# Elyptos/VolumetricRaytracer

Hardware: AMD Instinct MI355X
Metric: Mrays/sec at 1080p, 256^3 SDF volume (higher is better)
Workload: dtype f32

## Files before the change

include/vrt.h:

```cpp
#ifndef VRT_H
#define VRT_H

#include <stddef.h>
#include <stdint.h>

#ifdef __cplusplus
extern "C" {
#endif

#define VRT_MAX_VOLUMES      20
#define VRT_MAX_POINT_LIGHTS 5
#define VRT_MAX_SPOT_LIGHTS  5
#define VRT_MAX_INSTANCES    64
#define VRT_MAX_DEVICES      8
#define VRT_MAX_RESOLUTION   9
#define VRT_FRAMES_IN_FLIGHT 3
#define VRT_MAX_TEXTURES     64
#define VRT_FLAG_DIAG_TIMELINE 4
#define VRT_FLAG_OUTPUT_RGBA8 8

#define VRT_FLAG_BLOCK_PER_FRAME 64
#define VRT_FLAG_NO_CULL_RECT 128
#define VRT_FLAG_FULL_ONE_KERNEL 256
#define VRT_FLAG_FULL_THREE_PASS 512
#define VRT_FLAG_OUTPUT_BGRA8 2048
#define VRT_FLAG_NO_HIT_POLISH 1024
#define VRT_FLAG_REFERENCE_VIEW_VECTOR 4096
#define VRT_FLAG_REFERENCE_BOUNDARY_TEXELS 8192
#define VRT_HIT_POLISH_SAMPLES 2
#define VRT_FLAG_NO_TIMING 16

enum vrt_status {
    VRT_OK = 0,
    VRT_ERR_INVALID = -1,
    VRT_ERR_NO_DEVICE = -2,
    VRT_ERR_HIP = -3,
    VRT_ERR_OOM = -4,
    VRT_ERR_SLOT = -5,
    VRT_ERR_NOT_READY = -6,
    VRT_ERR_UNSUPPORTED = -7
};

enum vrt_render_mode {
// ... 244 lines not shown

int vrt_last_timing(vrt_ctx* ctx, vrt_timing* out);
int vrt_timing_history(vrt_ctx* ctx, int n, float* kernel_ms_out);

int vrt_launch_history(vrt_ctx* ctx, int n, float* kernel_ms_out, int* frames_out);

long long vrt_debug_wave_records(vrt_ctx* ctx, int which, uint32_t* out, long long max_words);

#define VRT_FORM_FULL 1
#define VRT_FORM_PASSES 2
#define VRT_FORM_TEXTURED 4
#define VRT_FORM_MAY_BOUNCE 8
#define VRT_FORM_LEAN_REF 16
int vrt_debug_last_kernel_form(vrt_ctx* ctx);

int vrt_debug_gather_ceiling(vrt_ctx* ctx, int format, int coherent_lanes, unsigned n_bricks, float* gsamples_per_s_out);

const char* vrt_strerror(int status);
const char* vrt_version(void);

#ifdef __cplusplus
}
#endif
#endif
```

volumetricraytracer_amd/_abi.py:

```python
from __future__ import annotations

import ctypes as C
import os

VRT_MAX_VOLUMES = 20
VRT_MAX_TEXTURES = 64
VRT_FRAMES_IN_FLIGHT = 3
VRT_MAX_RESOLUTION = 9
VRT_MAX_POINT_LIGHTS = 5
VRT_MAX_SPOT_LIGHTS = 5
VRT_MAX_INSTANCES = 64
VRT_MAX_DEVICES = 8
VRT_COMM_ID_BYTES = 128

VRT_OK = 0
VRT_ERR_INVALID = -1
VRT_ERR_NO_DEVICE = -2
VRT_ERR_HIP = -3
VRT_ERR_OOM = -4
VRT_ERR_SLOT = -5
VRT_ERR_NOT_READY = -6
VRT_ERR_UNSUPPORTED = -7

MODE_INTERP = 0
# ... 4 lines not shown
MODE_CUBE_UNLIT = 5
MODE_CUBE_NOTEX = 6
MODE_CUBE_NOTEX_UNLIT = 7

FORM_FULL, FORM_PASSES, FORM_TEXTURED, FORM_MAY_BOUNCE, FORM_LEAN_REF = 1, 2, 4, 8, 16
FLAG_DIAG_TIMELINE = 4
FLAG_OUTPUT_RGBA8 = 8
FLAG_NO_TIMING = 16
FLAG_BLOCK_PER_FRAME = 64
FLAG_NO_CULL_RECT = 128
FLAG_FULL_ONE_KERNEL = 256
FLAG_FULL_THREE_PASS = 512
FLAG_OUTPUT_BGRA8 = 2048
FLAG_REFERENCE_VIEW_VECTOR = 4096
FLAG_REFERENCE_BOUNDARY_TEXELS = 8192
FLAG_NO_HIT_POLISH = 1024
HIT_POLISH_SAMPLES = 2
MAX_BLOCK_FRAMES = 48
MAX_LAUNCH_FRAMES = 256

VOLUME_BYTES_DENSE, VOLUME_BYTES_MATERIAL, VOLUME_BYTES_BRICKS, VOLUME_BYTES_CELLS = 0, 1, 2, 3
VOLUME_BYTES_SKIP, VOLUME_BYTES_NIB, VOLUME_BYTES_CUBE_SKIP, VOLUME_BYTES_ACTIVE_BOX = 4, 5, 6, 7

FORMAT_F32 = 0
FORMAT_TEXEL16 = 1

PATH_AUTO = 0
PATH_DENSE = 1
PATH_BRICK = 2
PATH_BRICK_LDS = 3
# ... 191 lines not shown
    "vrt_comm_init": (C.c_int, [C.c_void_p, C.c_int, C.c_int, C.c_void_p]),
    "vrt_comm_destroy": (C.c_int, [C.c_void_p]),
    "vrt_comm_expect_sizes": (C.c_int, [C.c_void_p, C.c_size_t, C.c_size_t]),
    "vrt_gather_tiles": (C.c_int, [C.c_void_p, C.c_void_p, C.c_void_p, C.c_size_t, C.c_int, C.c_void_p]),
    "vrt_exchange_tiles": (C.c_int, [C.c_void_p, C.c_void_p, C.c_void_p, C.c_size_t, C.c_void_p]),
    "vrt_render_begin": (C.c_int, [C.c_void_p, C.POINTER(vrt_params), C.c_int]),
    "vrt_render_end": (C.c_int, [C.c_void_p, C.c_int, C.POINTER(C.c_void_p)]),
    "vrt_trace_rays": (C.c_int, [C.c_void_p, C.POINTER(vrt_params), C.c_int, C.c_int, C.c_void_p, C.c_void_p, C.c_void_p]),
    "vrt_trace_rays_host": (C.c_int, [C.c_void_p, C.POINTER(vrt_params), C.c_int, C.c_int, C.c_void_p, C.c_void_p]),
    "vrt_camera_rays": (C.c_int, [C.POINTER(vrt_scene), C.c_int, C.c_int, C.c_int, C.c_void_p, C.c_void_p]),
    "vrt_last_timing": (C.c_int, [C.c_void_p, C.POINTER(vrt_timing)]),
    "vrt_timing_history": (C.c_int, [C.c_void_p, C.c_int, C.POINTER(C.c_float)]),
    "vrt_launch_history": (C.c_int, [C.c_void_p, C.c_int, C.POINTER(C.c_float), C.POINTER(C.c_int)]),
    "vrt_debug_wave_records": (C.c_longlong, [C.c_void_p, C.c_int, C.c_void_p, C.c_longlong]),
    "vrt_debug_last_kernel_form": (C.c_int, [C.c_void_p]),
    "vrt_debug_gather_ceiling": (C.c_int, [C.c_void_p, C.c_int, C.c_int, C.c_uint, C.POINTER(C.c_float)]),
    "vrt_strerror": (C.c_char_p, [C.c_int]),
    "vrt_version": (C.c_char_p, []),
}

LIB_PATH = os.path.join(os.path.dirname(os.path.abspath(__file__)), "lib", "libvrt_hip.so")

_lib = None


def _share_hip_runtime_with_torch() -> None:
    import sys

    if "torch" in sys.modules or os.environ.get("VRT_NO_TORCH_PRELOAD") == "1":
        return
# ... 42 lines not shown
```

volumetricraytracer_amd/csrc/host/HipRenderer.cpp:

```cpp
#include "HipRenderer.h"

#include <algorithm>

#include <cmath>
#include <cstdio>
#include <cstdlib>
#include <cstring>
#include <vector>

#include <zlib.h>

#define V_LOG_ERROR(msg) fprintf(stderr, "[VHipRenderer][error] %s\n", (msg))
#define V_LOG_WARNING(msg) fprintf(stderr, "[VHipRenderer][warning] %s\n", (msg))

namespace VolumeRaytracer {

VObjectPtr<VTexture2D> VTexture2D::LoadPPM(const std::string& path) {
    FILE* f = fopen(path.c_str(), "rb");
    if (!f) return nullptr;
    auto token = [&](char* buf, size_t n) {
        int c = fgetc(f);
        while (c != EOF) {
            if (c == '#') {
                while (c != EOF && c != '\n') c = fgetc(f);
// ... 579 lines not shown
    p.max_steps = MaxSteps << std::max(0, MaxResolution - 8);
    p.shadow = Shadows ? 1 : 0;
    p.mode = (int)RenderMode;
    p.path = DataPath;
    p.max_bounces = MaxBounces;
    p.eps_hit = std::min(0.004f * MinCell, 0.02f);
    p.eps_in = 0.01f;
    p.step_min = std::min(0.004f * MinCell, 0.02f);
    p.k_relax = Relaxation;
    const VObjectPtr<Scene::VCamera> cam = scene.GetActiveCamera();
    p.cone_eps = std::tan((cam ? cam->FOVAngle : 60.f) * (3.14159265358979323846f / 180.0f) * 0.5f) / (float)Height;
    if (FrameFormat != EFrameFormat::Float4) p.flags |= VRT_FLAG_OUTPUT_RGBA8;
    if (FrameFormat == EFrameFormat::BGRA8) p.flags |= VRT_FLAG_OUTPUT_BGRA8;
    if (ReferenceViewVector) p.flags |= VRT_FLAG_REFERENCE_VIEW_VECTOR;
    if (ReferenceBoundaryTexels) p.flags |= VRT_FLAG_REFERENCE_BOUNDARY_TEXELS;
    return p;
}

void VHipRenderer::Render() {
    if (!IsActive()) {
        V_LOG_WARNING("Render() on an inactive renderer");
        return;
    }
    const VObjectPtr<Scene::VScene> scene = SceneRef.lock();
    if (!scene) return;
    if (const VObjectPtr<Scene::VCamera> cam = scene->GetActiveCamera()) cam->AspectRatio = (float)Width / (float)Height;
    if (!SyncWithScene(*scene)) return;
    const vrt_params p = MakeParams(*scene);
    const size_t bytes = (size_t)Width * Height * BytesPerPixel();
    if (FramesInFlight <= 1 || Devices.size() != 1) {
// ... 174 lines not shown
```

volumetricraytracer_amd/csrc/host/HipRenderer.h:

```cpp
#pragma once
#include <functional>
#include <map>
#include <string>
#include <vector>
#include "../../../include/vrt.h"
#include "HostRenderer.h"

namespace VolumeRaytracer {
namespace Renderer {
namespace Hip {

class VHipRenderer : public VRenderer {
public:
    VHipRenderer();
    ~VHipRenderer() override;

    void Render() override;
    bool Start() override;
    void Stop() override;
    bool IsActive() const override { return Ctx != nullptr; }
    void InitializeTexture(VObjectPtr<VTexture> texture) override;
    void UploadToGPU(VObjectPtr<VTexture> texture) override;
    void UploadToGPU(VObjectPtr<VTextureCube> texture);
    void UploadToGPU(VObjectPtr<VTexture2D> texture);
// ... 5 lines not shown
    enum class EFrameFormat { Float4, RGBA8, BGRA8 };
    EFrameFormat FrameFormat = EFrameFormat::BGRA8;
    size_t BytesPerPixel() const { return FrameFormat == EFrameFormat::Float4 ? 16 : 4; }
    const void* GetFrameData() const { return FramePixels; }
    size_t GetFrameByteCount() const { return FrameBytes; }
    const float* GetFramePixels() const { return FrameFormat == EFrameFormat::Float4 ? static_cast<const float*>(FramePixels) : nullptr; }
    unsigned GetWidth() const { return Width; }
    unsigned GetHeight() const { return Height; }
    bool GetLastTiming(vrt_timing& out) const;
    int MaxSteps = 255;
    int VolumeFormat = VRT_FORMAT_TEXEL16;
    bool RegionUploads = true;
    bool ReferenceDefaultTextures = true;
    bool ReferenceViewVector = true;
    bool ReferenceBoundaryTexels = true;
    float Relaxation = 1.7f;
    bool Shadows = true;
    int MaxBounces = 2;
    int DataPath = VRT_PATH_AUTO;
    int FramesInFlight = 3;
    void Flush();
    bool RenderBlock(int n_frames, const std::function<void(int)>& tick);
    const void* GetBlockFrame(int f) const { return (BlockFrames && f >= 0 && f < BlockFrameCount) ? BlockFrames + (size_t)f * BlockFrameBytes : nullptr; }
    bool TraceRays(const std::vector<vrt_ray>& rays, std::vector<vrt_hit>& hits, bool anyHit = false);
    bool Pick(int px, int py, vrt_hit& out);
    const Scene::VVoxelObject* HitObject(const vrt_hit& hit) const {
        return hit.instance >= 0 && (size_t)hit.instance < QueryObjects.size() ? QueryObjects[(size_t)hit.instance] : nullptr;
    }

    bool ApplyBrushes(const Scene::VVoxelObject& object, const std::vector<vrt_brush>& brushes, vrt_brush_result* result = nullptr);
// ... 43 lines not shown
```

volumetricraytracer_amd/csrc/vrt_api.hip:

```cpp
#include <hip/hip_runtime.h>

#include <dlfcn.h>
#include <math.h>
#include <stdio.h>
#include <string.h>

#include <algorithm>
#include <chrono>
#include <limits>
#include <new>
#include <vector>

#include "../../include/vrt.h"
#include "vrt_device.h"
#include "vrt_launch.h"
#include "voxelize_core.h"

using namespace vrt;

namespace {

constexpr int kNcclUint8 = 1;
struct RcclApi {
    typedef struct { char internal[VRT_COMM_ID_BYTES]; } UniqueId;
// ... 148 lines not shown
    unsigned* d_diag = nullptr;
    void* edit_staging = nullptr;
    size_t edit_staging_cap = 0;
    void* edit_scratch = nullptr;
    size_t edit_scratch_cap = 0;
    int* d_box6 = nullptr;
    DBrushSlot* d_brush = nullptr;
    void* fill_scratch = nullptr;
    size_t fill_scratch_cap = 0;
    void* query_buf = nullptr;
    size_t query_cap = 0;
    int last_blocks = 0;
    int last_frames = 1;
    bool last_diag = false;
    int last_form = 0;
    hipEvent_t joined = nullptr;
    hipEvent_t ev0[kRing];
    hipEvent_t ev1[kRing];
    FrameSlot slot[VRT_FRAMES_IN_FLIGHT];
    bool events_ok = false;
    int ring_frames[kRing] = {};
    bool timed[kRing] = {};
};

}

struct vrt_ctx {
    std::vector<DeviceState> dev;
    HostVolume vol[VRT_MAX_VOLUMES];
    HostTexture tex[VRT_MAX_TEXTURES];
// ... 805 lines not shown
    }
    return VRT_OK;
}

int check_params(const vrt_ctx* ctx, const vrt_params* p, bool own_scenes = false) {
    if (!ctx || !p) return VRT_ERR_INVALID;
    if (p->width <= 0 || p->height <= 0 || p->width > 16384 || p->height > 16384) return VRT_ERR_INVALID;
    if (p->max_steps < 0 || p->max_steps > 65535 || p->max_bounces < 0 || p->max_bounces > 2) return VRT_ERR_INVALID;
    if (!(p->eps_hit == p->eps_hit) || !(p->step_min > 0.0f) || !(p->k_relax > 0.0f) || !(p->eps_in >= 0.0f) ||
        !(p->cone_eps >= 0.0f))
        return VRT_ERR_INVALID;
    if (p->mode < VRT_MODE_INTERP || p->mode > VRT_MODE_CUBE_NOTEX_UNLIT) return VRT_ERR_INVALID;
    if (p->path < VRT_PATH_AUTO || p->path > VRT_PATH_CELLS) return VRT_ERR_INVALID;
    if ((p->flags & ~(3 | VRT_FLAG_DIAG_TIMELINE | VRT_FLAG_OUTPUT_RGBA8 | VRT_FLAG_NO_TIMING | 32 | VRT_FLAG_BLOCK_PER_FRAME | VRT_FLAG_NO_CULL_RECT |
                      VRT_FLAG_FULL_ONE_KERNEL | VRT_FLAG_FULL_THREE_PASS | VRT_FLAG_NO_HIT_POLISH | VRT_FLAG_OUTPUT_BGRA8 |
                      VRT_FLAG_REFERENCE_VIEW_VECTOR | VRT_FLAG_REFERENCE_BOUNDARY_TEXELS)) != 0 || (p->flags & 3) == 3 ||
        ((p->flags & VRT_FLAG_OUTPUT_BGRA8) && !(p->flags & VRT_FLAG_OUTPUT_RGBA8)) ||
        ((p->flags & VRT_FLAG_FULL_ONE_KERNEL) && (p->flags & VRT_FLAG_FULL_THREE_PASS)))
        return VRT_ERR_INVALID;
    if (!ctx->have_scene && !own_scenes) return VRT_ERR_NOT_READY;
    return VRT_OK;
}

int resolve_path(const vrt_ctx* ctx, int path, bool single, int mode, const vrt_scene* scenes = nullptr, int n_scenes = 0) {
    int n16 = 0, n32 = 0;
    if (!scenes) {
        scenes = &ctx->scene;
        n_scenes = 1;
    }
    for (int f = 0; f < n_scenes; f++)
        for (int i = 0; i < scenes[f].n_instances; i++)
// ... 151 lines not shown
                  : 0;
    F.back = p->mode >= VRT_MODE_CUBE ? 0.2f : 0.1f;
    F.max_bounces = p->max_bounces;
    F.width = p->width;
    F.height = p->height;
    F.row0 = row0;
    F.rows = rows;
    F.tiles_x = (p->width + 15) / 16;
    F.tiles_y = (rows + 15) / 16;
    F.tile_map = p->flags & 3;
    F.diag = (p->flags & VRT_FLAG_DIAG_TIMELINE) ? 1 : 0;
    F.rgba8 = (p->flags & VRT_FLAG_OUTPUT_RGBA8) ? ((p->flags & VRT_FLAG_OUTPUT_BGRA8) ? 2 : 1) : 0;
    F.polish = (p->flags & VRT_FLAG_NO_HIT_POLISH) ? 0 : VRT_HIT_POLISH_SAMPLES;
    F.view_vec = (p->flags & VRT_FLAG_REFERENCE_VIEW_VECTOR) ? 1 : 0;
    F.zero_outside = (p->flags & VRT_FLAG_REFERENCE_BOUNDARY_TEXELS) ? 1 : 0;
    F.strip_rows = rs.strip_rows;
    F.strip_first = rs.strip_first;
    F.strip_stride = rs.strip_stride;
    const ClosestHitForm form = closest_hit_form(ctx, p, scenes, n_scenes);
    F.textured = form.textured ? 1 : 0;
    F.full = form.full ? 1 : 0;
    F.may_bounce = form.may_bounce ? 1 : 0;
    F.n_inst = ctx->scene.n_instances;
    F.n_nodes = ctx->n_nodes;
    F.n_point = std::min(ctx->scene.n_point_lights, VRT_MAX_POINT_LIGHTS);
    F.n_spot = std::min(ctx->scene.n_spot_lights, VRT_MAX_SPOT_LIGHTS);
    F.vols = snapshot ? snapshot->vols : D.d_vols;
    F.inst = snapshot ? snapshot->inst : D.d_inst;
    F.nodes = snapshot ? snapshot->nodes : D.d_nodes;
    F.point = snapshot ? snapshot->point : D.d_point;
// ... 119 lines not shown
    if (passes) {
        const size_t per_frame = (size_t)D.last_blocks * 256, records = per_frame * (size_t)n_frames;
        if (per_frame > 0xffffffffull) return VRT_ERR_INVALID;
        if (D.pass_cap[slot] < records) {
            void* grown = nullptr;
            HIP_TRY(hipMalloc(&grown, records * (sizeof(HitRecord) + sizeof(unsigned)) + records / 64 * sizeof(unsigned long long)));
            if (D.d_pass[slot]) D.pass_retired.push_back(D.d_pass[slot]);
            D.d_pass[slot] = grown;
            D.pass_cap[slot] = records;
        }
        char* base = static_cast<char*>(D.d_pass[slot]);
        F.hit_rec = reinterpret_cast<HitRecord*>(base);
        F.hit_mask = reinterpret_cast<unsigned long long*>(base + D.pass_cap[slot] * sizeof(HitRecord));
        F.hit_aux = reinterpret_cast<unsigned*>(base + D.pass_cap[slot] * sizeof(HitRecord) + D.pass_cap[slot] / 64 * sizeof(unsigned long long));
        F.rec_stride = (uint32_t)per_frame;
    }
    D.last_diag = F.diag != 0;
    D.last_form = (F.full ? VRT_FORM_FULL : 0) | (passes ? VRT_FORM_PASSES : 0) | (F.textured ? VRT_FORM_TEXTURED : 0) |
                  (F.may_bounce ? VRT_FORM_MAY_BOUNCE : 0) | ((!F.full && (F.textured || F.view_vec || F.zero_outside)) ? VRT_FORM_LEAN_REF : 0);
    if (F.diag) {
        if (stat_blocks > (size_t)kMaxBlocks) return VRT_ERR_INVALID;
        if (!D.d_diag) HIP_TRY(hipMalloc(&D.d_diag, sizeof(unsigned) * kDiagRecord * 4 * (size_t)kMaxBlocks));
        F.diag_buf = D.d_diag;
    }
    hipStreamCaptureStatus cap = hipStreamCaptureStatusNone;
    if (stream != nullptr && hipStreamIsCapturing(stream, &cap) != hipSuccess) cap = hipStreamCaptureStatusNone;
    D.timed[ring] = cap == hipStreamCaptureStatusNone && !(p->flags & VRT_FLAG_NO_TIMING);
    D.ring_frames[ring] = n_frames;
    if (D.timed[ring]) HIP_TRY(hipEventRecord(D.ev0[ring], stream));
    HIP_TRY(launch_march(B, path, single, stream));
// ... 958 lines not shown
    } while (false);
    if (e0) (void)hipEventDestroy(e0);
    if (e1) (void)hipEventDestroy(e1);
    if (pool) (void)hipFree(pool);
    if (out) (void)hipFree(out);
    if (rc != VRT_OK) return rc;
    *gsamples_per_s_out = (float)((double)blocks * 256.0 * iters / ((double)best * 1e6));
    return VRT_OK;
}

int vrt_debug_last_kernel_form(vrt_ctx* ctx) {
    if (!ctx || ctx->dev.empty()) return VRT_ERR_INVALID;
    return ctx->dev[0].last_form;
}

long long vrt_debug_wave_records(vrt_ctx* ctx, int which, uint32_t* out, long long max_words) {
    if (!ctx || max_words < 0 || (max_words > 0 && !out) || which < 0 || which > 3) return VRT_ERR_INVALID;
    if (ctx->launches == 0) return VRT_ERR_NOT_READY;
    DeviceState& D = ctx->dev[0];
    const bool diag = (which & 1) != 0, whole = which >= 2;
    if (diag && (!D.last_diag || !D.d_diag)) return VRT_ERR_NOT_READY;
    const long long frame_words = (long long)D.last_blocks * 4 * (diag ? kDiagRecord : kStatRecord);
    const long long words = whole ? frame_words * D.last_frames : frame_words;
    if (out && max_words > 0) {
        HIP_TRY(hipSetDevice(D.ordinal));
        HIP_TRY(hipDeviceSynchronize());
        const uint32_t* src = (diag ? D.d_diag : D.d_stats[D.last_slot]) + (whole ? 0 : (size_t)(D.last_frames - 1) * (size_t)frame_words);
        HIP_TRY(hipMemcpy(out, src, sizeof(uint32_t) * (size_t)std::min(words, max_words), hipMemcpyDeviceToHost));
    }
    return words;
// ... 20 lines not shown
```

volumetricraytracer_amd/csrc/vrt_device.h:

```cpp
#pragma once
#include <stdint.h>

namespace vrt {

constexpr int kBrickCells = 4;
constexpr int kBrickSamples = 5;
constexpr int kBrickFloats = 128;
constexpr int kPathCube = 8;
constexpr int kPathBrick16 = 9;
constexpr int kPathCube16 = 10;
constexpr int kPathCells16 = 11;
constexpr int kNibWindow = 16;
constexpr int kTile = 8;
constexpr int kBlockThreads = 256;
constexpr int kMaxBvhNodes = 2 * 64 - 1;
constexpr int kStatWords = 7;
constexpr int kStatRecord = 8;
constexpr int kDiagRecord = 8;
constexpr int kMaxBlocks = 1 << 20;
#ifndef VRT_MAX_BLOCK_FRAMES
#define VRT_MAX_BLOCK_FRAMES 48
#endif
constexpr int kMaxBlockFrames = VRT_MAX_BLOCK_FRAMES;
constexpr int kMaxLaunchFrames = 256;
// ... 120 lines not shown
    unsigned* stats;
    unsigned* diag_buf;
    uint64_t frame_stride;
    uint32_t stats_stride;
    int32_t n_frames;
    const DVolume* vol0;
    HitRecord* hit_rec;
    unsigned* hit_aux;
    unsigned long long* hit_mask;
    const DCam* cams;
    uint32_t rec_stride;
    int32_t may_bounce;
    int32_t view_vec;
    int32_t zero_outside;
    const void* dyn;
};

struct DDyn {
    float light_dir[3];
    float light_strength;
    int32_t n_inst, n_nodes, n_point, n_spot;
    int32_t vol0_slot;
    int32_t pad_[7];
};
constexpr int kDynMaxInstances = 64;
constexpr int kDynMaxNodes = 128;
constexpr int kDynMaxPointLights = 5;
constexpr int kDynMaxSpotLights = 5;
static_assert(kDynMaxNodes >= kMaxBvhNodes, "a frame's BVH fits its section");
constexpr uint32_t kDynInstOff = sizeof(DDyn);
constexpr uint32_t kDynNodesOff = kDynInstOff + kDynMaxInstances * sizeof(DInstance);
constexpr uint32_t kDynPointOff = kDynNodesOff + kDynMaxNodes * sizeof(DBvhNode);
constexpr uint32_t kDynSpotOff = kDynPointOff + kDynMaxPointLights * sizeof(DPointLight);
constexpr uint32_t kDynStride = (kDynSpotOff + kDynMaxSpotLights * sizeof(DSpotLight) + 63u) & ~63u;
static_assert(sizeof(DDyn) == 64 && kDynStride % 64 == 0, "frame sections stay 64-byte aligned");

struct DBlock {
    DFrame f;
    DCam cam[kMaxBlockFrames];
};
static_assert(sizeof(DCam) == 64, "DCam is one s_load_dwordx16");
static_assert(sizeof(DBlock) <= 4096, "HIP kernarg segment limit");

}
```

volumetricraytracer_amd/csrc/vrt_kernels.hip:

```cpp
#include <hip/hip_runtime.h>
#include <math.h>
#include <stdlib.h>
#include "vrt_device.h"
#include "vrt_launch.h"
#include "voxelize_core.h"

namespace vrt {

struct F3 {
    float x, y, z;
};
__device__ __forceinline__ F3 f3(float x, float y, float z) { return F3{x, y, z}; }
__device__ __forceinline__ F3 operator+(F3 a, F3 b) { return f3(a.x + b.x, a.y + b.y, a.z + b.z); }
__device__ __forceinline__ F3 operator-(F3 a, F3 b) { return f3(a.x - b.x, a.y - b.y, a.z - b.z); }
__device__ __forceinline__ F3 operator*(F3 a, float s) { return f3(a.x * s, a.y * s, a.z * s); }
__device__ __forceinline__ float dot3(F3 a, F3 b) { return (a.x * b.x + a.y * b.y) + a.z * b.z; }
__device__ __forceinline__ F3 normalize3(F3 a) {
    float inv = 1.0f / sqrtf(dot3(a, a));
    return a * inv;
}
__device__ __forceinline__ float maxf_(float a, float b) { return a > b ? a : b; }
__device__ __forceinline__ float minf_(float a, float b) { return a < b ? a : b; }
__device__ __forceinline__ F3 mul33(const float* m, F3 v) {
    return f3((m[0] * v.x + m[1] * v.y) + m[2] * v.z, (m[3] * v.x + m[4] * v.y) + m[5] * v.z,
// ... 711 lines not shown
    if (!st.hit) {
        if (F.max_steps > 0 && st.i >= F.max_steps && !(st.t > R.t_end)) ex += kExhaustedOne;
        return false;
    }
    float t = st.t;
    Cell c = st.c;
    if (st.s_hit < 0.0f && st.i > 0) t = refine_hit<DP>(V, R, st.t_prev, st.s_prev, t, st.s_hit, c, steps);
    else if (NORMAL != 0 && F.polish > 0 && st.i > 0) t = polish_hit<DP>(F, V, R, t, st.s_hit, st.t_prev, st.s_prev, F.polish, c, steps);
    t_hit = t;
    if constexpr (NORMAL == 1) n_world = hit_normal<DP, false, REF>(I, V, R, c, st.i, REF && F.zero_outside != 0);
    if constexpr (NORMAL == 2) n_world = hit_normal<DP, true, REF>(I, V, R, c, st.i, REF && F.zero_outside != 0);
    return true;
    }
}

template <int PATH, bool SINGLE, bool DIAG = false, int NORMAL = 1, bool REF = false>
__device__ __forceinline__ bool trace_closest(const DFrame& F, F3 o, F3 d, float t_max, float t_base, float& t_best,
                                              int& inst_best, F3& n_best, unsigned& steps, unsigned& ex, DiagAcc* dg = nullptr) {
    if constexpr (SINGLE) {
        float t;
        F3 n;
        if (march_instance<PATH, NORMAL, DIAG, false, REF>(F, F.inst, F.vol0, o, d, t_max, t_base, t, n, steps, ex, dg)) {
            t_best = t;
            inst_best = 0;
            n_best = n;
            return true;
        }
        return false;
    } else {
        bool any = false;
        float best = t_max;
        int ni = 0;
        while (ni < F.n_nodes) {
            ni = __builtin_amdgcn_readfirstlane(ni);
            const DBvhNode nd = F.nodes[ni];
            const bool in = slab_box(o, d, nd, best);
            if (__ballot(in) == 0ull) {
// ... 14 lines not shown
                            t_best = t;
                            inst_best = ii;
                            n_best = n;
                        }
                    }
                }
                ni = nd.right;
            } else {
                ni = ni + 1;
            }
        }
        return any;
    }
}

template <int PATH, bool SINGLE, bool DIAG = false, bool DIR_SHADOW = false>
__device__ __forceinline__ bool trace_any(const DFrame& F, F3 o, F3 d, float t_max, float t_base, unsigned& steps, unsigned& ex,
                                          DiagAcc* dg = nullptr) {
    float t;
    F3 n;
    if constexpr (SINGLE) {
        return march_instance<PATH, 0, DIAG, DIR_SHADOW>(F, F.inst, F.vol0, o, d, t_max, t_base, t, n, steps, ex, dg);
    } else {
        bool found = false;
        int ni = 0;
        while (ni < F.n_nodes) {
            if (__ballot(!found) == 0ull) break;
            ni = __builtin_amdgcn_readfirstlane(ni);
            const DBvhNode nd = F.nodes[ni];
            const bool in = !found && slab_box(o, d, nd, t_max);
            if (__ballot(in) == 0ull) {
                ni = nd.right;
                continue;
            }
            if (nd.left < 0) {
                const DInstance* I = F.inst + (-nd.left - 1);
                if (in && march_instance<PATH, 0, DIAG, DIR_SHADOW, false, true>(F, I, F.vols + I->slot, o, d, t_max, t_base, t, n, steps, ex, dg)) found = true;
// ... 394 lines not shown
        const F3 t = tri_sample<CONST_ONLY>(V, 0, op, blend, false);
        albedo = f3(albedo.x * t.x, albedo.y * t.y, albedo.z * t.z);
    }
    if (V->tex_px[2] != nullptr) {
        const F3 t = tri_sample<CONST_ONLY>(V, 2, op, blend, false);
        rough = minf_(maxf_(V->roughness_raw * t.x, 0.0f), 1.0f);
        metal = minf_(maxf_(V->metallic_raw * t.y, 0.0f), 1.0f);
    }
    if (V->tex_px[1] != nullptr) {
        F3 t = tri_sample<CONST_ONLY>(V, 1, op, blend, true);
        t = normalize3(t);
        n = mul33(I->o2w, rotate_vector(f3(t.z, t.x, t.y), quat_from_x(no)));
    }
}

template <int PATH, bool SINGLE, bool DIAG, bool DYN = false,
          bool REF = false >
#ifndef VRT_BVH_WAVES
#define VRT_BVH_WAVES 7
#endif
__global__ __launch_bounds__(kMarchThreads) __attribute__((amdgpu_waves_per_eu((!SINGLE && !DIAG && PATH != VRT_PATH_DENSE) ? VRT_BVH_WAVES : (REF && SINGLE) ? 8 : 1))) void march_kernel(const DBlock B) {
    unsigned long long t_start = 0;
    if constexpr (DIAG) t_start = __builtin_amdgcn_s_memrealtime();
    const int frame = (int)blockIdx.y;
    DFrame Fd;
    const DFrame& F = frame_view<DYN>(B, frame, Fd);
    const DCam C = load_cam(B, frame);
    int b, wave;
    block_and_wave(b, wave);
    int tile_x, tile_y;
    tile_of_block(F, b, (int)gridDim.x / kMarchGridMul, tile_x, tile_y);
    const int lane = (int)threadIdx.x & 63;
    int px, pyl;
    pixel_of_lane(tile_x, tile_y, wave, lane, px, pyl);
    const int py = frame_row(F, pyl);
    const bool valid = tile_x < F.tiles_x && tile_y < F.tiles_y && px < F.width && pyl < F.rows && py < F.height;

    Counters k;
    DiagAcc dg;
    const bool reach = wave_can_reach(C, valid, px, py);

    if (valid) {
        F3 o, d;
        camera_ray(F, C, px, py, o, d);
        k.n_primary = 1;
        float t_hit = 0.0f;
        int inst = 0;
        F3 n = f3(0.0f, 0.0f, 0.0f);
        F3 color;
        const unsigned sky = env_fetch(F.env, F.env_size, d);
        if (reach && trace_closest<PATH, SINGLE, DIAG, 2, REF>(F, o, d, 10000.0f, 0.0f, t_hit, inst, n, k.s_primary, k.n_hits, &dg)) {
            k.n_hits += 1;
            bool shadowed = false;
            const F3 ld = f3(F.light_dir[0], F.light_dir[1], F.light_dir[2]);
            if constexpr (REF) {
                const DVolume* V = SINGLE ? F.vol0 : F.vols + F.inst[inst].slot;
                F3 albedo = f3(V->tint[0], V->tint[1], V->tint[2]);
                float rough = V->roughness, metal = V->metallic;
                if (F.textured) {
                    const F3 hp = f3(__builtin_fmaf(d.x, t_hit, o.x), __builtin_fmaf(d.y, t_hit, o.y), __builtin_fmaf(d.z, t_hit, o.z));
                    textured_surface<true>(V, SINGLE ? F.inst : F.inst + inst, hp, albedo, n, rough, metal);
                }
                if (F.shadow && !F.unlit && dot3(n, ld) > 0.0f) {
                    k.n_shadow = 1;
                    const float vs = F.view_vec ? camera_len(F, C, px, py) : 1.0f;
                    shadowed = trace_any<PATH, SINGLE, DIAG, true>(F, shadow_origin(F, o, d, t_hit, vs), ld, 5000.0f, t_hit, k.s_shadow, k.n_hits, &dg);
                }
                const float vs = F.view_vec ? camera_len(F, C, px, py) : 1.0f;
                color = shade_hit_surface(F, V, d, vs, n, albedo, rough, metal, shadowed);
            } else {
            if (F.shadow && !F.unlit && dot3(n, ld) > 0.0f) {
                k.n_shadow = 1;
                shadowed = trace_any<PATH, SINGLE, DIAG, true>(F, shadow_origin(F, o, d, t_hit), ld, 5000.0f, t_hit, k.s_shadow, k.n_hits, &dg);
            }
            color = shade_hit(F, SINGLE ? F.vol0 : F.vols + F.inst[inst].slot, d, n, shadowed);
            }
        } else {
            color = env_decode(sky);
        }
        store_pixel(F, frame, (unsigned)pyl * (unsigned)F.width + (unsigned)px, color);
    }
    write_records<DIAG, true>(F, frame, b, wave, lane, k, dg, t_start);
}

constexpr int kMaxDepth = 3;

#ifndef VRT_FULL_WAVES
#define VRT_FULL_WAVES 1
#endif
__device__ __forceinline__ size_t pass_record(const DFrame& F, int frame, int b, int wave, int lane) {
// ... 1387 lines not shown
```

volumetricraytracer_amd/renderer.py:

```python
from __future__ import annotations

import ctypes as C
from typing import Dict, List, Optional, Sequence

import numpy as np

from . import _abi
from .scene import VScene, VVoxelVolume, default_params, march_budget


RAY_DTYPE = np.dtype([("origin", "<f4", 3), ("t_max", "<f4"), ("direction", "<f4", 3), ("reserved_", "<f4")])
HIT_DTYPE = np.dtype([("t", "<f4"), ("normal", "<f4", 3), ("instance", "<i4"), ("voxel", "<i4", 3), ("material", "<u4"),
                      ("steps", "<u4"), ("reserved_", "<u4", 2)])
assert RAY_DTYPE.itemsize == C.sizeof(_abi.vrt_ray) and HIT_DTYPE.itemsize == C.sizeof(_abi.vrt_hit)


def make_rays(origins, directions, t_max=10000.0) -> np.ndarray:
    o = np.asarray(origins, dtype=np.float32).reshape(-1, 3)
    d = np.asarray(directions, dtype=np.float32).reshape(-1, 3)
    if len(o) != len(d):
        raise ValueError("origins and directions differ in length")
    rays = np.zeros(len(o), RAY_DTYPE)
    rays["origin"], rays["direction"] = o, d
    rays["t_max"] = np.broadcast_to(np.asarray(t_max, dtype=np.float32), (len(o),))
# ... 32 lines not shown
        self._lib = _abi.load()
        self._devices = list(devices)
        self._ctx = C.c_void_p()
        self._scene: Optional[VScene] = None
        self._slots: List[VVoxelVolume] = []
        self._uploaded: Dict[int, int] = {}
        self.RenderMode = _abi.MODE_INTERP
        self.Width, self.Height = 1024, 576
        self.params_override: Optional[_abi.vrt_params] = None
        self.DataPath = _abi.PATH_AUTO
        self.Shadows = True
        self.MaxSteps = 255
        self.MaxBounces = 2
        self.ReferenceViewVector = False
        self.ReferenceBoundaryTexels = False
        self._env_id = None
        self._tex_ids: Dict[int, int] = {}
        self._tex_keep: Dict[int, np.ndarray] = {}
        self._bound_tex: Dict[int, tuple] = {}

    def Start(self) -> bool:
        if self._ctx:
            return True
        arr = (C.c_int * len(self._devices))(*self._devices)
        rc = self._lib.vrt_create(C.byref(self._ctx), len(self._devices), arr)
        if rc != _abi.VRT_OK:
            print(f"[VHipRenderer] Start failed: {self._lib.vrt_strerror(rc).decode()}")
            self._ctx = C.c_void_p()
            return False
        return True
# ... 186 lines not shown
        self._tex_keep[key] = image
        return tid

    def make_params(self) -> _abi.vrt_params:
        if self.params_override is not None:
            p = _abi.vrt_params.from_buffer_copy(self.params_override)
        else:
            cell = min((v.GetCellSize() for v in self._scene.volumes()), default=1.0) if self._scene else 1.0
            res = max((v.Resolution for v in self._scene.volumes()), default=0) if self._scene else 0
            p = default_params(self.Width, self.Height, cell, max_steps=march_budget(res, self.MaxSteps), shadow=self.Shadows)
            p.max_bounces = self.MaxBounces
            if self.ReferenceViewVector:
                p.flags |= _abi.FLAG_REFERENCE_VIEW_VECTOR
            if self.ReferenceBoundaryTexels:
                p.flags |= _abi.FLAG_REFERENCE_BOUNDARY_TEXELS
        p.width, p.height = self.Width, self.Height
        p.mode = self.RenderMode
        if self.params_override is None:
            p.path = self.DataPath
        return p

    def render_rows(self, params: _abi.vrt_params, row0: int, rows: int, device_ptr: int, stream: int = 0) -> None:
        self._require()
        _abi.check(self._lib.vrt_render_rows(self._ctx, C.byref(params), row0, rows, C.c_void_p(device_ptr),
                                             C.c_void_p(stream)), "vrt_render_rows")

    def render_strips(self, params: _abi.vrt_params, strip_rows: int, first_strip: int, strip_stride: int, n_strips: int,
                      device_ptr: int, stream: int = 0) -> None:
        self._require()
        _abi.check(self._lib.vrt_render_strips(self._ctx, C.byref(params), strip_rows, first_strip, strip_stride, n_strips,
# ... 148 lines not shown
        return [(ms[i], fr[i]) for i in range(m)]

    def gather_ceiling(self, fmt: int = _abi.FORMAT_F32, coherent_lanes: bool = False, n_bricks: int = 32) -> float:
        self._require()
        out = C.c_float()
        _abi.check(self._lib.vrt_debug_gather_ceiling(self._ctx, int(fmt), 1 if coherent_lanes else 0, int(n_bricks), C.byref(out)), "vrt_debug_gather_ceiling")
        return float(out.value)

    def last_kernel_form(self) -> int:
        self._require()
        f = self._lib.vrt_debug_last_kernel_form(self._ctx)
        if f < 0:
            _abi.check(f, "vrt_debug_last_kernel_form")
        return int(f)

    def wave_records(self, which: int = 0) -> np.ndarray:
        self._require()
        n = self._lib.vrt_debug_wave_records(self._ctx, which, None, 0)
        if n < 0:
            _abi.check(int(n), "vrt_debug_wave_records")
        buf = np.zeros(int(n), dtype=np.uint32)
        self._lib.vrt_debug_wave_records(self._ctx, which, buf.ctypes.data_as(C.c_void_p), int(n))
        return buf.reshape(-1, 8)

    def _require(self) -> None:
        if not self._ctx:
            raise RuntimeError("renderer is not active (Start() not called or failed)")

    def __enter__(self):
        if not self.Start():
# ... 12 lines not shown
```

Baseline: 64910.

## Let in-reach waves adopt sky-only tiles so culled waves exit immediately

Adds a sky-adoption plan: when the camera's cull rectangle covers a meaningful fraction of the frame, waves whose tiles cannot reach geometry return at once, and waves inside the reach rectangle additionally fill sky pixels and records for culled tiles in strided order. This removes the launch and scheduling cost of many trivially-sky waves but lengthens in-reach waves and changes load balance. It also routes single-instance scene record pointers through the constant address space so loads can be scalar. A flag and a debug query allow disabling and inspecting the plan.

```diff
diff --git a/include/vrt.h b/include/vrt.h
--- a/include/vrt.h
+++ b/include/vrt.h
@@ -27,6 +27,7 @@
 #define VRT_FLAG_NO_HIT_POLISH 1024
 #define VRT_FLAG_REFERENCE_VIEW_VECTOR 4096
 #define VRT_FLAG_REFERENCE_BOUNDARY_TEXELS 8192
+#define VRT_FLAG_NO_SKY_ADOPTION 16384
 #define VRT_HIT_POLISH_SAMPLES 2
 #define VRT_FLAG_NO_TIMING 16
 
@@ -301,6 +302,8 @@
 #define VRT_FORM_LEAN_REF 16
 int vrt_debug_last_kernel_form(vrt_ctx* ctx);
 
+int vrt_debug_last_sky_adoption(vrt_ctx* ctx, int32_t* last_frame_plan);
+
 int vrt_debug_gather_ceiling(vrt_ctx* ctx, int format, int coherent_lanes, unsigned n_bricks, float* gsamples_per_s_out);
 
 const char* vrt_strerror(int status);
diff --git a/volumetricraytracer_amd/_abi.py b/volumetricraytracer_amd/_abi.py
--- a/volumetricraytracer_amd/_abi.py
+++ b/volumetricraytracer_amd/_abi.py
@@ -42,6 +42,7 @@
 FLAG_OUTPUT_BGRA8 = 2048
 FLAG_REFERENCE_VIEW_VECTOR = 4096
 FLAG_REFERENCE_BOUNDARY_TEXELS = 8192
+FLAG_NO_SKY_ADOPTION = 16384
 FLAG_NO_HIT_POLISH = 1024
 HIT_POLISH_SAMPLES = 2
 MAX_BLOCK_FRAMES = 48
@@ -263,6 +264,7 @@
     "vrt_launch_history": (C.c_int, [C.c_void_p, C.c_int, C.POINTER(C.c_float), C.POINTER(C.c_int)]),
     "vrt_debug_wave_records": (C.c_longlong, [C.c_void_p, C.c_int, C.c_void_p, C.c_longlong]),
     "vrt_debug_last_kernel_form": (C.c_int, [C.c_void_p]),
+    "vrt_debug_last_sky_adoption": (C.c_int, [C.c_void_p, C.POINTER(C.c_int32)]),
     "vrt_debug_gather_ceiling": (C.c_int, [C.c_void_p, C.c_int, C.c_int, C.c_uint, C.POINTER(C.c_float)]),
     "vrt_strerror": (C.c_char_p, [C.c_int]),
     "vrt_version": (C.c_char_p, []),
diff --git a/volumetricraytracer_amd/csrc/host/HipRenderer.cpp b/volumetricraytracer_amd/csrc/host/HipRenderer.cpp
--- a/volumetricraytracer_amd/csrc/host/HipRenderer.cpp
+++ b/volumetricraytracer_amd/csrc/host/HipRenderer.cpp
@@ -617,6 +617,7 @@
     if (FrameFormat == EFrameFormat::BGRA8) p.flags |= VRT_FLAG_OUTPUT_BGRA8;
     if (ReferenceViewVector) p.flags |= VRT_FLAG_REFERENCE_VIEW_VECTOR;
     if (ReferenceBoundaryTexels) p.flags |= VRT_FLAG_REFERENCE_BOUNDARY_TEXELS;
+    if (!SkyAdoption) p.flags |= VRT_FLAG_NO_SKY_ADOPTION;
     return p;
 }
 
diff --git a/volumetricraytracer_amd/csrc/host/HipRenderer.h b/volumetricraytracer_amd/csrc/host/HipRenderer.h
--- a/volumetricraytracer_amd/csrc/host/HipRenderer.h
+++ b/volumetricraytracer_amd/csrc/host/HipRenderer.h
@@ -43,6 +43,7 @@
     bool ReferenceDefaultTextures = true;
     bool ReferenceViewVector = true;
     bool ReferenceBoundaryTexels = true;
+    bool SkyAdoption = true;
     float Relaxation = 1.7f;
     bool Shadows = true;
     int MaxBounces = 2;
diff --git a/volumetricraytracer_amd/csrc/vrt_api.hip b/volumetricraytracer_amd/csrc/vrt_api.hip
--- a/volumetricraytracer_amd/csrc/vrt_api.hip
+++ b/volumetricraytracer_amd/csrc/vrt_api.hip
@@ -186,6 +186,8 @@
     int last_frames = 1;
     bool last_diag = false;
     int last_form = 0;
+    int last_adopted = 0;
+    SkyAdopt last_plan = {};
     hipEvent_t joined = nullptr;
     hipEvent_t ev0[kRing];
     hipEvent_t ev1[kRing];
@@ -1021,7 +1023,7 @@
     if (p->path < VRT_PATH_AUTO || p->path > VRT_PATH_CELLS) return VRT_ERR_INVALID;
     if ((p->flags & ~(3 | VRT_FLAG_DIAG_TIMELINE | VRT_FLAG_OUTPUT_RGBA8 | VRT_FLAG_NO_TIMING | 32 | VRT_FLAG_BLOCK_PER_FRAME | VRT_FLAG_NO_CULL_RECT |
                       VRT_FLAG_FULL_ONE_KERNEL | VRT_FLAG_FULL_THREE_PASS | VRT_FLAG_NO_HIT_POLISH | VRT_FLAG_OUTPUT_BGRA8 |
-                      VRT_FLAG_REFERENCE_VIEW_VECTOR | VRT_FLAG_REFERENCE_BOUNDARY_TEXELS)) != 0 || (p->flags & 3) == 3 ||
+                      VRT_FLAG_REFERENCE_VIEW_VECTOR | VRT_FLAG_REFERENCE_BOUNDARY_TEXELS | VRT_FLAG_NO_SKY_ADOPTION)) != 0 || (p->flags & 3) == 3 ||
         ((p->flags & VRT_FLAG_OUTPUT_BGRA8) && !(p->flags & VRT_FLAG_OUTPUT_RGBA8)) ||
         ((p->flags & VRT_FLAG_FULL_ONE_KERNEL) && (p->flags & VRT_FLAG_FULL_THREE_PASS)))
         return VRT_ERR_INVALID;
@@ -1203,6 +1205,7 @@
     F.polish = (p->flags & VRT_FLAG_NO_HIT_POLISH) ? 0 : VRT_HIT_POLISH_SAMPLES;
     F.view_vec = (p->flags & VRT_FLAG_REFERENCE_VIEW_VECTOR) ? 1 : 0;
     F.zero_outside = (p->flags & VRT_FLAG_REFERENCE_BOUNDARY_TEXELS) ? 1 : 0;
+    F.sky_adopt = (!(p->flags & VRT_FLAG_NO_SKY_ADOPTION) && F.tile_map == kMapSupertile && rs.strip_rows == 0 && row0 == 0 && rows == p->height) ? 1 : 0;
     F.strip_rows = rs.strip_rows;
     F.strip_first = rs.strip_first;
     F.strip_stride = rs.strip_stride;
@@ -1352,6 +1355,15 @@
         F.hit_mask = reinterpret_cast<unsigned long long*>(base + D.pass_cap[slot] * sizeof(HitRecord));
         F.hit_aux = reinterpret_cast<unsigned*>(base + D.pass_cap[slot] * sizeof(HitRecord) + D.pass_cap[slot] / 64 * sizeof(unsigned long long));
         F.rec_stride = (uint32_t)per_frame;
+    }
+    D.last_adopted = 0;
+    for (int f = 0; f < n_frames && F.sky_adopt && !F.full && !F.diag && single; f++) {
+        const DCam& c = device_cams ? D.h_cams[slot][f] : B.cam[f];
+        D.last_adopted += sky_adopt_plan(F.width, F.rows, c.cull_lo, c.cull_hi).on ? 1 : 0;
+    }
+    {
+        const DCam& c = device_cams ? D.h_cams[slot][n_frames - 1] : B.cam[n_frames - 1];
+        D.last_plan = sky_adopt_plan(F.width, F.rows, c.cull_lo, c.cull_hi);
     }
     D.last_diag = F.diag != 0;
     D.last_form = (F.full ? VRT_FORM_FULL : 0) | (passes ? VRT_FORM_PASSES : 0) | (F.textured ? VRT_FORM_TEXTURED : 0) |
@@ -2340,6 +2352,17 @@
     return ctx->dev[0].last_form;
 }
 
+int vrt_debug_last_sky_adoption(vrt_ctx* ctx, int32_t* last_frame_plan) {
+    if (!ctx || ctx->dev.empty()) return VRT_ERR_INVALID;
+    const DeviceState& D = ctx->dev[0];
+    if (last_frame_plan) {
+        const SkyAdopt& A = D.last_plan;
+        const int32_t v[6] = {A.rx0, A.ry0, A.rx1, A.ry1, A.n_reach, A.n_culled};
+        memcpy(last_frame_plan, v, sizeof v);
+    }
+    return D.last_adopted;
+}
+
 long long vrt_debug_wave_records(vrt_ctx* ctx, int which, uint32_t* out, long long max_words) {
     if (!ctx || max_words < 0 || (max_words > 0 && !out) || which < 0 || which > 3) return VRT_ERR_INVALID;
     if (ctx->launches == 0) return VRT_ERR_NOT_READY;
diff --git a/volumetricraytracer_amd/csrc/vrt_device.h b/volumetricraytracer_amd/csrc/vrt_device.h
--- a/volumetricraytracer_amd/csrc/vrt_device.h
+++ b/volumetricraytracer_amd/csrc/vrt_device.h
@@ -158,6 +158,8 @@
     int32_t view_vec;
     int32_t zero_outside;
     const void* dyn;
+    int32_t sky_adopt;
+    int32_t pad_;
 };
 
 struct DDyn {
@@ -179,6 +181,36 @@
 constexpr uint32_t kDynStride = (kDynSpotOff + kDynMaxSpotLights * sizeof(DSpotLight) + 63u) & ~63u;
 static_assert(sizeof(DDyn) == 64 && kDynStride % 64 == 0, "frame sections stay 64-byte aligned");
 
+constexpr int kSkyAdoptMax = 2;
+struct SkyAdopt {
+    bool on;
+    int wx_n, wy_n;
+    int rx0, ry0, rx1, ry1;
+    int rw;
+    int n_reach, n_culled;
+    int n_top, side, n_mid;
+};
+__host__ __device__ __attribute__((always_inline)) inline SkyAdopt sky_adopt_plan(int width, int rows, uint32_t cull_lo, uint32_t cull_hi) {
+    SkyAdopt A;
+    A.on = false;
+    A.wx_n = A.wy_n = A.rx0 = A.ry0 = A.rx1 = A.ry1 = A.rw = A.n_reach = A.n_culled = A.n_top = A.side = A.n_mid = 0;
+    const int x0 = (int)(cull_lo & 0xffffu), y0 = (int)(cull_lo >> 16), x1 = (int)(cull_hi & 0xffffu), y1 = (int)(cull_hi >> 16);
+    const int xe = x1 < width - 1 ? x1 : width - 1, ye = y1 < rows - 1 ? y1 : rows - 1;
+    if (x0 > xe || y0 > ye) return A;
+    A.wx_n = (width + kTile - 1) / kTile;
+    A.wy_n = (rows + kTile - 1) / kTile;
+    A.rx0 = x0 / kTile; A.ry0 = y0 / kTile; A.rx1 = xe / kTile; A.ry1 = ye / kTile;
+    A.rw = A.rx1 - A.rx0 + 1;
+    const int rh = A.ry1 - A.ry0 + 1;
+    A.n_reach = A.rw * rh;
+    A.n_culled = A.wx_n * A.wy_n - A.n_reach;
+    A.n_top = A.ry0 * A.wx_n;
+    A.side = A.wx_n - A.rw;
+    A.n_mid = rh * A.side;
+    A.on = A.n_culled > 0 && A.n_culled <= kSkyAdoptMax * A.n_reach;
+    return A;
+}
+
 struct DBlock {
     DFrame f;
     DCam cam[kMaxBlockFrames];
diff --git a/volumetricraytracer_amd/csrc/vrt_kernels.hip b/volumetricraytracer_amd/csrc/vrt_kernels.hip
--- a/volumetricraytracer_amd/csrc/vrt_kernels.hip
+++ b/volumetricraytracer_amd/csrc/vrt_kernels.hip
@@ -749,13 +749,20 @@
     }
 }
 
-template <int PATH, bool SINGLE, bool DIAG = false, int NORMAL = 1, bool REF = false>
+template <class T>
+__device__ __forceinline__ const T* scene_record(const T* p) {
+    const __attribute__((address_space(4))) T* c = (const __attribute__((address_space(4))) T*)p;
+    asm("" : "+s"(c));
+    return (const T*)c;
+}
+
+template <int PATH, bool SINGLE, bool DIAG = false, int NORMAL = 1, bool REF = false, bool CONST_SCENE = false >
 __device__ __forceinline__ bool trace_closest(const DFrame& F, F3 o, F3 d, float t_max, float t_base, float& t_best,
                                               int& inst_best, F3& n_best, unsigned& steps, unsigned& ex, DiagAcc* dg = nullptr) {
     if constexpr (SINGLE) {
         float t;
         F3 n;
-        if (march_instance<PATH, NORMAL, DIAG, false, REF>(F, F.inst, F.vol0, o, d, t_max, t_base, t, n, steps, ex, dg)) {
+        if (march_instance<PATH, NORMAL, DIAG, false, REF>(F, CONST_SCENE ? scene_record(F.inst) : F.inst, CONST_SCENE ? scene_record(F.vol0) : F.vol0, o, d, t_max, t_base, t, n, steps, ex, dg)) {
             t_best = t;
             inst_best = 0;
             n_best = n;
@@ -800,13 +807,13 @@
     }
 }
 
-template <int PATH, bool SINGLE, bool DIAG = false, bool DIR_SHADOW = false>
+template <int PATH, bool SINGLE, bool DIAG = false, bool DIR_SHADOW = false, bool CONST_SCENE = false>
 __device__ __forceinline__ bool trace_any(const DFrame& F, F3 o, F3 d, float t_max, float t_base, unsigned& steps, unsigned& ex,
                                           DiagAcc* dg = nullptr) {
     float t;
     F3 n;
     if constexpr (SINGLE) {
-        return march_instance<PATH, 0, DIAG, DIR_SHADOW>(F, F.inst, F.vol0, o, d, t_max, t_base, t, n, steps, ex, dg);
+        return march_instance<PATH, 0, DIAG, DIR_SHADOW>(F, CONST_SCENE ? scene_record(F.inst) : F.inst, CONST_SCENE ? scene_record(F.vol0) : F.vol0, o, d, t_max, t_base, t, n, steps, ex, dg);
     } else {
         bool found = false;
         int ni = 0;
@@ -1231,12 +1238,37 @@
     }
 }
 
+__device__ __forceinline__ void sky_adopt_tile(const SkyAdopt& A, int c, int& ax, int& ay) {
+    if (c < A.n_top) {
+        ay = (int)((unsigned)c / (unsigned)A.wx_n);
+        ax = c - ay * A.wx_n;
+    } else if (c - A.n_top < A.n_mid) {
+        const int m = c - A.n_top, row = (int)((unsigned)m / (unsigned)A.side), i = m - row * A.side;
+        ay = A.ry0 + row;
+        ax = i < A.rx0 ? i : i + A.rw;
+    } else {
+        const int m = c - A.n_top - A.n_mid, row = (int)((unsigned)m / (unsigned)A.wx_n);
+        ay = A.ry1 + 1 + row;
+        ax = m - row * A.wx_n;
+    }
+}
+__device__ __forceinline__ void block_of_wave_tile(const DFrame& F, int ax, int ay, int& b, int& wave) {
+    const int tx = ax >> 1, ty = ay >> 1;
+    wave = (ax & 1) | ((ay & 1) << 1);
+    const int st_x = (F.tiles_x + 3) >> 2;
+    const int st = (ty >> 2) * st_x + (tx >> 2);
+    const int within = (tx & 3) | ((ty & 3) << 2);
+    const int q = ((st >> 3) << 4) | within;
+    b = (q << 3) | ((st - (int)blockIdx.y) & 7);
+}
+
 template <int PATH, bool SINGLE, bool DIAG, bool DYN = false,
           bool REF = false >
 #ifndef VRT_BVH_WAVES
 #define VRT_BVH_WAVES 7
 #endif
 __global__ __launch_bounds__(kMarchThreads) __attribute__((amdgpu_waves_per_eu((!SINGLE && !DIAG && PATH != VRT_PATH_DENSE) ? VRT_BVH_WAVES : (REF && SINGLE) ? 8 : 1))) void march_kernel(const DBlock B) {
+    constexpr bool kAdopt = SINGLE && !DIAG;
     unsigned long long t_start = 0;
     if constexpr (DIAG) t_start = __builtin_amdgcn_s_memrealtime();
     const int frame = (int)blockIdx.y;
@@ -1256,6 +1288,37 @@
     Counters k;
     DiagAcc dg;
     const bool reach = wave_can_reach(C, valid, px, py);
+    if constexpr (kAdopt) {
+        const __attribute__((address_space(4))) void* kp = (const __attribute__((address_space(4))) void*)__builtin_amdgcn_kernarg_segment_ptr();
+        asm volatile("" : "+s"(kp));
+        const DFrame& FA = *(const DFrame*)kp;
+        SkyAdopt A;
+        A.on = false;
+        if (FA.sky_adopt) A = sky_adopt_plan(FA.width, FA.rows, C.cull_lo, C.cull_hi);
+        if (A.on) {
+            const int wx = tile_x * 2 + (wave & 1), wy = tile_y * 2 + (wave >> 1);
+            if (!reach) {
+                if (wx < A.wx_n && wy < A.wy_n) return;
+            } else {
+                for (int c = (wy - A.ry0) * A.rw + (wx - A.rx0); c < A.n_culled; c += A.n_reach) {
+                    int ax, ay;
+                    sky_adopt_tile(A, c, ax, ay);
+                    const int apx = ax * kTile + (lane & 7), apyl = ay * kTile + (lane >> 3);
+                    const bool avalid = apx < FA.width && apyl < FA.rows;
+                    Counters ak;
+                    if (avalid) {
+                        F3 o, d;
+                        camera_ray(FA, C, apx, frame_row(FA, apyl), o, d);
+                        ak.n_primary = 1;
+                        store_pixel(FA, frame, (unsigned)apyl * (unsigned)FA.width + (unsigned)apx, env_decode(env_fetch(FA.env, FA.env_size, d)));
+                    }
+                    int ab, awave;
+                    block_of_wave_tile(FA, ax, ay, ab, awave);
+                    write_records<false, true>(FA, frame, ab, awave, lane, ak, dg, 0ull);
+                }
+            }
+        }
+    }
 
     if (valid) {
         F3 o, d;
@@ -1266,31 +1329,31 @@
         F3 n = f3(0.0f, 0.0f, 0.0f);
         F3 color;
         const unsigned sky = env_fetch(F.env, F.env_size, d);
-        if (reach && trace_closest<PATH, SINGLE, DIAG, 2, REF>(F, o, d, 10000.0f, 0.0f, t_hit, inst, n, k.s_primary, k.n_hits, &dg)) {
+        if (reach && trace_closest<PATH, SINGLE, DIAG, 2, REF, kAdopt>(F, o, d, 10000.0f, 0.0f, t_hit, inst, n, k.s_primary, k.n_hits, &dg)) {
             k.n_hits += 1;
             bool shadowed = false;
             const F3 ld = f3(F.light_dir[0], F.light_dir[1], F.light_dir[2]);
             if constexpr (REF) {
-                const DVolume* V = SINGLE ? F.vol0 : F.vols + F.inst[inst].slot;
+                const DVolume* V = kAdopt ? scene_record(F.vol0) : SINGLE ? F.vol0 : F.vols + F.inst[inst].slot;
                 F3 albedo = f3(V->tint[0], V->tint[1], V->tint[2]);
                 float rough = V->roughness, metal = V->metallic;
                 if (F.textured) {
                     const F3 hp = f3(__builtin_fmaf(d.x, t_hit, o.x), __builtin_fmaf(d.y, t_hit, o.y), __builtin_fmaf(d.z, t_hit, o.z));
-                    textured_surface<true>(V, SINGLE ? F.inst : F.inst + inst, hp, albedo, n, rough, metal);
+                    textured_surface<true>(V, kAdopt ? scene_record(F.inst) : SINGLE ? F.inst : F.inst + inst, hp, albedo, n, rough, metal);
                 }
                 if (F.shadow && !F.unlit && dot3(n, ld) > 0.0f) {
                     k.n_shadow = 1;
                     const float vs = F.view_vec ? camera_len(F, C, px, py) : 1.0f;
-                    shadowed = trace_any<PATH, SINGLE, DIAG, true>(F, shadow_origin(F, o, d, t_hit, vs), ld, 5000.0f, t_hit, k.s_shadow, k.n_hits, &dg);
+                    shadowed = trace_any<PATH, SINGLE, DIAG, true, kAdopt>(F, shadow_origin(F, o, d, t_hit, vs), ld, 5000.0f, t_hit, k.s_shadow, k.n_hits, &dg);
                 }
                 const float vs = F.view_vec ? camera_len(F, C, px, py) : 1.0f;
                 color = shade_hit_surface(F, V, d, vs, n, albedo, rough, metal, shadowed);
             } else {
             if (F.shadow && !F.unlit && dot3(n, ld) > 0.0f) {
                 k.n_shadow = 1;
-                shadowed = trace_any<PATH, SINGLE, DIAG, true>(F, shadow_origin(F, o, d, t_hit), ld, 5000.0f, t_hit, k.s_shadow, k.n_hits, &dg);
-            }
-            color = shade_hit(F, SINGLE ? F.vol0 : F.vols + F.inst[inst].slot, d, n, shadowed);
+                shadowed = trace_any<PATH, SINGLE, DIAG, true, kAdopt>(F, shadow_origin(F, o, d, t_hit), ld, 5000.0f, t_hit, k.s_shadow, k.n_hits, &dg);
+            }
+            color = shade_hit(F, kAdopt ? scene_record(F.vol0) : SINGLE ? F.vol0 : F.vols + F.inst[inst].slot, d, n, shadowed);
             }
         } else {
             color = env_decode(sky);
diff --git a/volumetricraytracer_amd/renderer.py b/volumetricraytracer_amd/renderer.py
--- a/volumetricraytracer_amd/renderer.py
+++ b/volumetricraytracer_amd/renderer.py
@@ -70,6 +70,7 @@
         self.MaxBounces = 2
         self.ReferenceViewVector = False
         self.ReferenceBoundaryTexels = False
+        self.SkyAdoption = True
         self._env_id = None
         self._tex_ids: Dict[int, int] = {}
         self._tex_keep: Dict[int, np.ndarray] = {}
@@ -286,6 +287,8 @@
                 p.flags |= _abi.FLAG_REFERENCE_VIEW_VECTOR
             if self.ReferenceBoundaryTexels:
                 p.flags |= _abi.FLAG_REFERENCE_BOUNDARY_TEXELS
+            if not self.SkyAdoption:
+                p.flags |= _abi.FLAG_NO_SKY_ADOPTION
         p.width, p.height = self.Width, self.Height
         p.mode = self.RenderMode
         if self.params_override is None:
@@ -464,6 +467,14 @@
             _abi.check(f, "vrt_debug_last_kernel_form")
         return int(f)
 
+    def last_sky_adoption(self):
+        self._require()
+        plan = (C.c_int32 * 6)()
+        n = self._lib.vrt_debug_last_sky_adoption(self._ctx, plan)
+        if n < 0:
+            _abi.check(n, "vrt_debug_last_sky_adoption")
+        return int(n), dict(zip(("rx0", "ry0", "rx1", "ry1", "n_reach", "n_culled"), (int(x) for x in plan)))
+
     def wave_records(self, which: int = 0) -> np.ndarray:
         self._require()
         n = self._lib.vrt_debug_wave_records(self._ctx, which, None, 0)
```

New measurement: 59080. 0.91x the previous value.
